# Michaelszeng/GCS-ADMM

Measured on NVIDIA B200. Metric: admm_iterations_per_second, higher is better.
Workload: dtype f64

## Files before the change

gcs-admm_b200/build.py:

```python
from __future__ import annotations

import os
import shutil
import subprocess
import sys

HERE = os.path.dirname(os.path.abspath(__file__))
SRC = os.path.join(HERE, "csrc", "gcsadmm.cu")


def deps():
    import glob
    return sorted(glob.glob(os.path.join(HERE, "csrc", "*.cu")) + glob.glob(os.path.join(HERE, "csrc", "*.cuh"))
                  + glob.glob(os.path.join(os.path.dirname(HERE), "include", "*.h")))


OUT = os.path.join(HERE, "libgcsadmm.so")


def nvcc_path():
    for cand in (shutil.which("nvcc"), "/usr/local/cuda/bin/nvcc"):
        if cand and os.path.exists(cand):
            return cand
    raise RuntimeError("nvcc not found: libgcsadmm.so cannot be built")


def build(force=False, verbose=False):
    if not force and os.path.exists(OUT) and all(os.path.getmtime(OUT) >= os.path.getmtime(d) for d in deps()):
        return OUT
    cmd = [nvcc_path(), "-gencode", "arch=compute_100a,code=sm_100a", "-lineinfo", "-O3", "-std=c++17",
           "-Xptxas", "-v", "-shared", "-Xcompiler", "-fPIC", "-ccbin", "/usr/bin/g++", "-o", OUT, SRC]
    r = subprocess.run(cmd, capture_output=True, text=True)
    if verbose or r.returncode != 0:
        sys.stderr.write(r.stdout + r.stderr)
    if r.returncode != 0:
        raise RuntimeError("nvcc failed building libgcsadmm.so")
    with open(os.path.join(HERE, "csrc", "ptxas_info.txt"), "w") as fh:
        fh.write(r.stderr)
    return OUT


if __name__ == "__main__":
    print(build(force=True, verbose=True))
```

gcs-admm_b200/csrc/gcsadmm.cu:

```cuda
#include <cuda_runtime.h>
#include <math.h>
#include <stdio.h>
#include <stdlib.h>
#include <string.h>
#include <new>
#include <nvtx3/nvToolsExt.h>

struct NvtxRange {
    explicit NvtxRange(const char *name) { nvtxRangePushA(name); }
    ~NvtxRange() { nvtxRangePop(); }
};

#include "../../include/gcsadmm.h"
#include "gcs_ctrl.h"
#include "vertex_update.cuh"
#include "vertex_perf.cuh"

#define GCS_VERSION "gcsadmm 0.1.0 (sm_100a)"
#define K1_MAX_WARPS 12
#define EDGE_THREADS 256

static thread_local char g_err[512] = "";
static int set_err(int code, const char *fmt, const char *a = "", const char *b = "") {
    snprintf(g_err, sizeof g_err, fmt, a, b);
// ... 68 lines not shown
vertex_kernel(GcsGraphView G, GcsStateView St, Ctrl *ctrl_all, const int *__restrict__ vprob, GcsScratchLayout L, double tol, int max_iter) {
    extern __shared__ double smem[];
    const int lane = threadIdx.x & 31, warp = threadIdx.x >> 5;
    const int v = blockIdx.x * (blockDim.x >> 5) + warp;
    if (v >= G.nV) return;
    Ctrl *ctrl = ctrl_all + (vprob ? vprob[v] : 0);
    if (ctrl->stop && !ctrl->ignore_stop) return;
    double *S = smem + (size_t)warp * L.total;
    int status = 0;
    const int iters = gcs_vertex_update(G, St, v, ctrl->rho, ctrl->mu_scale, tol, max_iter, L, S, lane, &status);
    if (lane == 0) {
        if (iters) atomicAdd(&ctrl->inner_iters, (unsigned long long)iters);
        if (status > 0 && status != 5) atomicAdd(&ctrl->inner_fail, 1);
        if (status < 0) atomicAdd(&ctrl->skipped, 1ull);
    }
}

__device__ __forceinline__ unsigned long long gcs_globaltimer() { unsigned long long t; asm volatile("mov.u64 %0, %globaltimer;" : "=l"(t)); return t; }

__device__ __forceinline__ void peer_push(const double *xc, const int *__restrict__ send_he, const int *__restrict__ send_rank,
                                          const int *__restrict__ send_slot, int nsend, const PeerView &PV) {
    const int k = PV.comm[PV.rank]->k + 1, par = k & 1;
    for (int i = threadIdx.x; i < 5 * nsend; i += blockDim.x) {
        const int j = i / 5, c = i - 5 * j, q = send_rank[j];
        PV.xc[q][5 * ((size_t)PV.nHown[q] + (size_t)par * PV.nHghost[q] + send_slot[j]) + c] = __ldcg(xc + 5 * (size_t)send_he[j] + c);
    }
    __threadfence_system();
    __syncthreads();
    if (threadIdx.x < PV.world && ((PV.neighbours >> threadIdx.x) & 1u)) *(volatile int *)&PV.comm[threadIdx.x]->halo_flag[PV.rank] = k;
}
__device__ __forceinline__ void peer_wait_halo(const PeerView &PV) {
    PeerComm *me = PV.comm[PV.rank];
    const int k = me->k + 1, p = threadIdx.x;
    if (p < PV.world && ((PV.neighbours >> p) & 1u)) {
        const unsigned long long t0 = gcs_globaltimer();
        while (*(volatile int *)&me->halo_flag[p] < k)
            if (gcs_globaltimer() - t0 > GCS_PEER_TIMEOUT_NS) { me->error = 1; break; }
        __threadfence_system();
    }
    __syncthreads();
}

template <bool INNER, bool BATCH>
__global__ void __launch_bounds__(GCS_PERF_THREADS, 4)
vertex_perf_kernel(GcsGraphView G, GcsStateView St, GcsPerfTables T, Ctrl *ctrl_all, GcsPerfLayout L, PeerPush P) {
    extern __shared__ __align__(16) double smem[];
    __shared__ __align__(8) unsigned long long bar[2];
    if (!BATCH) {
        if (ctrl_all->stop && !ctrl_all->ignore_stop) return;
        if (blockIdx.x == 0 && threadIdx.x == 0) atomicAdd(&ctrl_all->inner_iters, (unsigned long long)T.inner_iters * (unsigned long long)G.nV);
    }
    int tile = blockIdx.x;
    if (tile >= T.ntiles) return;
    double *const stage0 = smem + L.work;
#define STAGE(b) (stage0 + (b) * L.stage)
    if (threadIdx.x == 0) {
        gcs_mbar_init(&bar[0], 1);
        gcs_mbar_init(&bar[1], 1);
        gcs_perf_stage(T, L, STAGE(0), tile, &bar[0]);
    }
    __syncthreads();
    double rin = 0.0;
    for (unsigned n = 0; tile < T.ntiles; tile += gridDim.x, ++n) {
        const int buf = n & 1;
        gcs_mbar_wait(&bar[buf], (n >> 1) & 1u);
        gcs_perf_tile<INNER, BATCH>(G, St, T, L, smem, STAGE(buf), tile, ctrl_all, rin, STAGE(buf ^ 1), tile + gridDim.x, &bar[buf ^ 1]);
    }
    if (threadIdx.x == GCS_COPY_THREAD) gcs_bulk_wait_read();
#undef STAGE
    if (INNER) {
#pragma unroll
        for (int o = 16; o; o >>= 1) rin += __shfl_xor_sync(0xffffffffu, rin, o);
        __syncthreads();
        if ((threadIdx.x & 31) == 0) smem[L.rin + (threadIdx.x >> 5)] = rin;
        __syncthreads();
        if (threadIdx.x == 0) {
            double s = 0.0;
            for (int w2 = 0; w2 < (int)(blockDim.x >> 5); ++w2) s += smem[L.rin + w2];
            T.tile_res[blockIdx.x] = s;
        }
    }
    if (P.PV) {
        __shared__ int is_last;
        __threadfence();
        __syncthreads();
        if (threadIdx.x == 0) is_last = (atomicAdd(P.ticket, 1u) == gridDim.x - 1);
        __syncthreads();
        if (is_last) {
            __threadfence();
            peer_push(St.xc, P.send_he, P.send_rank, P.send_slot, P.nsend, *P.PV);
            if (threadIdx.x == 0) *P.ticket = 0u;
        }
    }
}
__global__ void perf_init_dead_kernel(GcsGraphView G, GcsStateView St) {
    const int v = blockIdx.x * blockDim.x + threadIdx.x;
    if (v >= G.nV || G.vtype[v] != GCS_VT_DEAD) return;
    for (int k = 0; k < 4; ++k) { St.z_v[4 * (size_t)v + k] = 0.0; St.x_v[4 * (size_t)v + k] = G.cent[2 * (size_t)v + (k & 1)]; }
    St.y_v[v] = 0.0;
}

__device__ void control_apply(Ctrl *ctrl, const GcsParams &p, long long n_x, long long n_mu, double *hist, int hist_cap) {
    const int it = ctrl->it + 1;
    const double *s = ctrl->sums;
    const double rho = ctrl->rho;
    const double pri = sqrt(s[0]);
    const double dual = rho * sqrt(2.0 * s[1]);
    double rho_new = rho, scale = 1.0;
    const bool may = it < p.frac * p.max_it && (p.adapt_every <= 1 || it % p.adapt_every == 0);
    if (pri >= p.nu * dual && may) { rho_new = rho * p.tau_incr; scale = 1.0 / p.tau_incr; }
    else if (dual >= p.nu * pri && may) { rho_new = rho * (1.0 / p.tau_decr); scale = p.tau_incr; }
    const double nAx = sqrt(s[2]), nBz = sqrt(2.0 * s[3]), nmu = scale * sqrt(s[4]);
    const double eps_pri = sqrt((double)n_x) * p.eps_abs + p.eps_rel * fmax(nAx, nBz);
    const double eps_dual = sqrt((double)n_mu) * p.eps_abs + p.eps_rel * nmu;
    const double inner = s[6] < 0.0 ? -1.0 : sqrt(s[6]);
    const double pri_g = s[7] < 0.0 ? -1.0 : sqrt(s[7]), dual_g = s[8] < 0.0 ? -1.0 : rho * sqrt(2.0 * s[8]);
    ctrl->pri_g = pri_g; ctrl->dual_g = dual_g;
    ctrl->it = it; ctrl->pri = pri; ctrl->dual = dual; ctrl->eps_pri = eps_pri; ctrl->eps_dual = eps_dual; ctrl->inner = inner;
    ctrl->rho = rho_new; ctrl->mu_scale = scale;
    if (it < hist_cap) { hist[it] = rho_new; hist[hist_cap + it] = pri; hist[2 * hist_cap + it] = dual; }
// ... 994 lines not shown
                        if (gb < g || (gb == 2) != (bb == c->blk_off[v + 1] - 1)) rc = set_err(GCS_E_INVALID, "perf-mode blocks of a vertex are not in-, out-, z-block order%s", "");
                        g = gb; nin += gb == 0;
                    }
                    int *w = vrec + GCS_VI_N * (size_t)v;
                    w[GCS_VI_CONE] = c->cone_off[v] - c->cone_off[a]; w[GCS_VI_NV] = c->cone_off[v + 1] - c->cone_off[v];
                    w[GCS_VI_CLS] = c->vclass[v]; w[GCS_VI_TERM] = (vtype[v] != GCS_VT_GENERIC) | (nin << 1);
                    w[GCS_VI_BLK] = c->blk_off[v] - c->blk_off[a]; w[GCS_VI_NB] = c->blk_off[v + 1] - c->blk_off[v];
                    w[GCS_VI_ACTIVE] = vprob[v]; w[GCS_VI_HE] = he_off[v] - he_off[a];
                }
            }
            if (!rc) rc = upload(&h->p_blk_rec, brec, 4 * nB);
            if (!rc) rc = upload(&h->p_vrec, vrec, GCS_VI_N * nVt);
            if (!rc) rc = upload(&h->p_tile_rec, trec, 8 * nT);
        }
        free(brec); free(vrec); free(trec); free(he_edge); free(he_off); free(vtype); free(he_flags); free(vprob);
    }
    if (!rc) rc = upload(&h->p_tstate, (const double *)nullptr, 12 * (size_t)c->n_blocks);
    if (!rc) rc = upload(&h->p_tn, (const double *)nullptr, 2 * (size_t)h->nV);
    if (!rc) rc = upload(&h->p_tile_res, (const double *)nullptr, (size_t)c->n_tiles);
    if (!rc && c->edge_delta) rc = upload(&h->p_edge_delta, c->edge_delta, 2 * (size_t)h->nE);
    if (!rc && c->edge_delta && c->edge_cent) rc = upload(&h->p_edge_cent, c->edge_cent, 2 * (size_t)h->nE);
    if (rc) { free_perf(h); return rc; }
    h->perf_nblocks = c->n_blocks;
    h->PL = gcs_perf_layout(c->cap_blocks, c->cap_verts, c->cap_cone);
    h->PT.vclass = h->p_vclass; h->PT.cls_tab = h->p_cls_tab; h->PT.cone_off = h->p_cone_off; h->PT.cone = h->p_cone;
    h->PT.blk_off = h->p_blk_off; h->PT.blk_rec = h->p_blk_rec; h->PT.vrec = h->p_vrec; h->PT.tile_rec = h->p_tile_rec;
    h->PT.ntiles = c->n_tiles; h->PT.tstate = h->p_tstate; h->PT.tn = h->p_tn; h->PT.inner_iters = c->inner_iters;
    h->PT.alpha = c->alpha; h->PT.kappa = c->kappa; h->PT.theta = c->theta > 0.0 ? c->theta : 1.0; h->PT.edge_delta = h->p_edge_delta; h->PT.tile_res = h->p_tile_res;
    cudaDeviceProp prop;
    CK(cudaGetDeviceProperties(&prop, h->device));
    const size_t bytes = (size_t)(h->PL.work + 2 * h->PL.stage) * sizeof(double);
    if (bytes > prop.sharedMemPerBlockOptin) { free_perf(h); return set_err(GCS_E_INVALID, "perf-mode tile too large for shared memory (a vertex of very high degree)%s", ""); }
    h->perf_smem = (int)bytes;
    h->perf_threads = c->threads >= 32 && c->threads <= GCS_PERF_THREADS ? (c->threads / 32) * 32 : GCS_PERF_THREADS;
    {
        const char *bps = getenv("GCS_PERF_BLOCKS_PER_SM");
        int per_sm = bps && atoi(bps) > 0 ? atoi(bps) : 4;
        const int by_smem = (int)(prop.sharedMemPerMultiprocessor / (bytes + 1024));
        if (per_sm > by_smem) per_sm = by_smem > 0 ? by_smem : 1;
        const long long cap = (long long)prop.multiProcessorCount * per_sm;
        h->perf_grid = (int)(c->n_tiles < cap ? c->n_tiles : cap);
    }
    for (auto *k : {vertex_perf_kernel<false, false>, vertex_perf_kernel<true, false>, vertex_perf_kernel<false, true>, vertex_perf_kernel<true, true>}) {
        CK(cudaFuncSetAttribute(k, cudaFuncAttributeMaxDynamicSharedMemorySize, h->perf_smem));
        CK(cudaFuncSetAttribute(k, cudaFuncAttributePreferredSharedMemoryCarveout, 100));
    }
    perf_init_dead_kernel<<<(h->nV + 255) / 256, 256, 0, h->stream>>>(graph_view(h), state_view(h));
    CK(cudaGetLastError());
    CK(cudaStreamSynchronize(h->stream));
    h->perf_on = 1;
    return 0;
}

extern "C" int gcsadmm_get_perf_state(GcsHandle *h, double *tstate, double *tn) {
    if (!h || !h->perf_on) return set_err(GCS_E_INVALID, "perf mode is not enabled%s", "");
    CK(cudaSetDevice(h->device));
    CK(cudaStreamSynchronize(h->stream));
    if (tstate && h->perf_nblocks) CK(cudaMemcpy(tstate, h->p_tstate, sizeof(double) * 12 * (size_t)h->perf_nblocks, cudaMemcpyDeviceToHost));
    if (tn) CK(cudaMemcpy(tn, h->p_tn, sizeof(double) * 2 * (size_t)h->nV, cudaMemcpyDeviceToHost));
    return 0;
}
extern "C" int gcsadmm_set_perf_state(GcsHandle *h, const double *tstate, const double *tn) {
    if (!h || !h->perf_on) return set_err(GCS_E_INVALID, "perf mode is not enabled%s", "");
    CK(cudaSetDevice(h->device));
    CK(cudaStreamSynchronize(h->stream));
    if (tstate && h->perf_nblocks) CK(cudaMemcpy(h->p_tstate, tstate, sizeof(double) * 12 * (size_t)h->perf_nblocks, cudaMemcpyHostToDevice));
    if (tn) CK(cudaMemcpy(h->p_tn, tn, sizeof(double) * 2 * (size_t)h->nV, cudaMemcpyHostToDevice));
    return 0;
}
```

gcs-admm_b200/csrc/vertex_perf.cuh:

```cuda
#pragma once
#include <string.h>
#include "gcs_ctrl.h"
#include "vertex_update.cuh"

#define GCS_CONE_REC 12
#define GCS_NCX 19
#define GCS_CLS_G0 361
#define GCS_CLS_DINV 380
#define GCS_CLS_STRIDE 392
#define GCS_PERF_THREADS 256

#ifdef GCS_EMULATE
#define GCS_CTA_LOOP(i, n) for (int i = 0; i < (n); ++i)
#define GCS_CTA_SYNC() ((void)0)
#else
#define GCS_CTA_LOOP(i, n) for (int i = threadIdx.x; i < (n); i += blockDim.x)
#define GCS_CTA_SYNC() __syncthreads()
#endif

struct GcsPerfTables {
    const int *vclass;
    const double *cls_tab;
    const int *cone_off;
    const double *cone;
// ... 102 lines not shown
        if (dist > 0.0) gcs_cone_take_face(gcs_cone_sector_dot(cone, k, 0, c0, c1, c2) >= 0.0 && gcs_cone_sector_dot(cone, k, 1, c0, c1, c2) >= 0.0, k, best, code, inside);
    }
    gcs_cone_pick(cone, code, inside, c0, c1, c2, q0, q1, q2);
}
GCS_DEV void gcs_cone_project2(const double *cone, int nv, double c0, double c1, double c2, double d0, double d1, double d2,
                               double &q0, double &q1, double &q2, double &s0, double &s1, double &s2) {
    double best_c = 0.0, best_d = 0.0;
    int code_c = -1, code_d = -1;
    bool inside_c = true, inside_d = true;
#pragma unroll 1
    for (int k = 0; k < nv; ++k) {
        const GcsConeRay R = gcs_cone_ray(cone, k);
        const double dist_c = gcs_cone_test_ray(R, k, c0, c1, c2, best_c, code_c);
        const double dist_d = gcs_cone_test_ray(R, k, d0, d1, d2, best_d, code_d);
        if (dist_c > 0.0 || dist_d > 0.0) {
            const bool ma_c = gcs_cone_sector_dot(cone, k, 0, c0, c1, c2) >= 0.0, ma_d = gcs_cone_sector_dot(cone, k, 0, d0, d1, d2) >= 0.0;
            const bool mb_c = gcs_cone_sector_dot(cone, k, 1, c0, c1, c2) >= 0.0, mb_d = gcs_cone_sector_dot(cone, k, 1, d0, d1, d2) >= 0.0;
            if (dist_c > 0.0) gcs_cone_take_face(ma_c && mb_c, k, best_c, code_c, inside_c);
            if (dist_d > 0.0) gcs_cone_take_face(ma_d && mb_d, k, best_d, code_d, inside_d);
        }
    }
    gcs_cone_pick(cone, code_c, inside_c, c0, c1, c2, q0, q1, q2);
    gcs_cone_pick(cone, code_d, inside_d, d0, d1, d2, s0, s1, s2);
}

#if !defined(GCS_EMULATE) && defined(__CUDACC__)
__device__ __forceinline__ unsigned gcs_smem_u32(const void *p) { return (unsigned)__cvta_generic_to_shared(p); }
__device__ __forceinline__ void gcs_mbar_init(unsigned long long *bar, unsigned count) {
    asm volatile("mbarrier.init.shared::cta.b64 [%0], %1;" ::"r"(gcs_smem_u32(bar)), "r"(count) : "memory");
    asm volatile("fence.mbarrier_init.release.cluster;" ::: "memory");
}
__device__ __forceinline__ void gcs_mbar_expect_tx(unsigned long long *bar, unsigned bytes) {
    asm volatile("mbarrier.arrive.expect_tx.shared::cta.b64 _, [%0], %1;" ::"r"(gcs_smem_u32(bar)), "r"(bytes) : "memory");
}
__device__ __forceinline__ void gcs_bulk_g2s(void *dst, const void *src, unsigned bytes, unsigned long long *bar) {
    asm volatile("cp.async.bulk.shared::cluster.global.mbarrier::complete_tx::bytes [%0], [%1], %2, [%3];"
                 ::"r"(gcs_smem_u32(dst)), "l"(src), "r"(bytes), "r"(gcs_smem_u32(bar)) : "memory");
}
__device__ __forceinline__ void gcs_mbar_wait(unsigned long long *bar, unsigned parity) {
    unsigned done = 0;
    while (!done) {
        asm volatile("{\n .reg .pred p;\n mbarrier.try_wait.parity.shared::cta.b64 p, [%1], %2;\n selp.u32 %0, 1, 0, p;\n}"
                     : "=r"(done) : "r"(gcs_smem_u32(bar)), "r"(parity) : "memory");
    }
}
__device__ __forceinline__ void gcs_bulk_s2g(void *dst, const void *src, unsigned bytes) {
    asm volatile("cp.async.bulk.global.shared::cta.bulk_group [%0], [%1], %2;" ::"l"(dst), "r"(gcs_smem_u32(src)), "r"(bytes) : "memory");
}
__device__ __forceinline__ void gcs_bulk_commit() { asm volatile("cp.async.bulk.commit_group;" ::: "memory"); }
__device__ __forceinline__ void gcs_bulk_wait_read() { asm volatile("cp.async.bulk.wait_group.read 0;" ::: "memory"); }
__device__ __forceinline__ void gcs_fence_async_smem() { asm volatile("fence.proxy.async.shared::cta;" ::: "memory"); }
#endif

#define GCS_PF 3

GCS_DEV double gcs_core_input(const double *tS, const double *rS, const int *w, int k, double kappa) {
    const int bl = w[GCS_VI_BLK], zb = bl + w[GCS_VI_NB] - 1;
    double s = 0.0;
    if (k < 4) {
        if (!(w[GCS_VI_TERM] & 1)) { for (int b = bl; b <= zb; ++b) s += tS[12 * b + 6 * (k >> 1) + 3 + (k & 1)]; s *= kappa; }
    } else if (k < 9) s = rS[5 * zb + k - 4];
    else {
        const int g = k >= 14, tau = k - 9 - 5 * g, bin = bl + (w[GCS_VI_TERM] >> 1);
        for (int b = g ? bin : bl; b < (g ? zb : bin); ++b) s += rS[5 * b + tau];
    }
    return s;
}
GCS_DEV double gcs_core_output(const double *tab, const double *in, int k) {
    const double *gk = tab + k;
    double s0 = tab[GCS_CLS_G0 + k], s1 = 0.0;
#pragma unroll
    for (int j = 0; j + 1 < GCS_NCX; j += 2) { s0 += gk[GCS_NCX * j] * in[j]; s1 += gk[GCS_NCX * (j + 1)] * in[j + 1]; }
    return s0 + s1 + gk[GCS_NCX * (GCS_NCX - 1)] * in[GCS_NCX - 1];
}

GCS_DEV double gcs_rhs(const GcsPerfTables &T, const double *tS, const double *TS, const double *tnS, const int *brec, int q, int vl, double rho, double kappa) {
    const int b = q / 5, tau = q - 5 * b, info = brec[4 * b + 1], grp = (info >> 8) & 3;
    const bool term = (info >> 10) & 1;
    const double *d = tS + 12 * b;
    double val;
    if (tau < 4) {
        const int i = tau >> 1, c = tau & 1;
        val = d[6 * i + c];
        if (!term) val -= d[6 * i + 3 + c];
        val *= kappa;
        if (grp == 1) val += TS[q];
        else if (grp == 0) { if (tau < 2) val += TS[q + 2]; }
        else val += (i ? -kappa : kappa) * tnS[2 * vl + c];
    } else {
        val = d[2] + d[8];
        if (!term) val += (1.0 - d[5]) + (1.0 - d[11]);
        val *= kappa;
        if (grp < 2) val += T.theta * TS[q] - GCS_EDGE_PENALTY / rho;
    }
    return val;
}
GCS_DEV double gcs_block_u(const double *rS, const double *co, const double *tab, int info, int b, int tau) {
    const int grp = (info >> 8) & 3;
    return grp == 2 ? co[4 + tau] : tab[GCS_CLS_DINV + 5 * grp + tau] * rS[5 * b + tau] + co[9 + 5 * grp + tau];
}

GCS_DEV double gcs_target_z(const GcsStateView &St, const GcsPerfTables &T, int e, int c, int info) {
    double zc = St.z[5 * (size_t)e + c];
    if (T.edge_delta && ((info >> 8) & 3) == 1 && (c == 2 || c == 3))
        zc -= T.edge_delta[2 * (size_t)e + c - 2] * St.z[5 * (size_t)e + 4];
    return zc;
}


#if !defined(GCS_EMULATE) && defined(__CUDACC__)
#define GCS_COPY_THREAD (blockDim.x - 32)
__device__ __forceinline__ void gcs_perf_stage(const GcsPerfTables &T, const GcsPerfLayout &L, double *B, int tile, unsigned long long *bar) {
    const int *tr = T.tile_rec + 8 * (size_t)tile;
    const int v0 = tr[0], nvt = tr[1], b0 = tr[2], nb = tr[3], c0 = tr[4], ncone = tr[5];
    gcs_mbar_expect_tx(bar, (unsigned)(sizeof(double) * (12 * nb + 2 * nvt + GCS_CONE_REC * ncone) + sizeof(int) * (GCS_VI_N * nvt + 4 * nb + 8)));
    gcs_bulk_g2s(B + L.tr, tr, (unsigned)(sizeof(int) * 8), bar);
    gcs_bulk_g2s(B + L.vi, T.vrec + GCS_VI_N * (size_t)v0, (unsigned)(sizeof(int) * GCS_VI_N * nvt), bar);
    if (nb) gcs_bulk_g2s(B + L.bi, T.blk_rec + 4 * (size_t)b0, (unsigned)(sizeof(int) * 4 * nb), bar);
    if (nb) gcs_bulk_g2s(B + L.tS, T.tstate + 12 * (size_t)b0, (unsigned)(sizeof(double) * 12 * nb), bar);
    gcs_bulk_g2s(B + L.tnS, T.tn + 2 * (size_t)v0, (unsigned)(sizeof(double) * 2 * nvt), bar);
    if (ncone) gcs_bulk_g2s(B + L.cone, T.cone + GCS_CONE_REC * (size_t)c0, (unsigned)(sizeof(double) * GCS_CONE_REC * ncone), bar);
}
#endif

GCS_DEV void gcs_cstep_store(double *t, double *e, double t0, double t1, double t2, double q0, double q1, double q2, double ms, double alpha) {
    const double l0 = ms * (t0 - q0), l1 = ms * (t1 - q1), l2 = ms * (t2 - q2);
    t[0] = q0 - l0; t[1] = q1 - l1; t[2] = q2 - l2;
    e[0] = (1.0 - alpha) * q0 + l0; e[1] = (1.0 - alpha) * q1 + l1; e[2] = (1.0 - alpha) * q2 + l2;
}

template <bool INNER, bool BATCH>
GCS_DEV void gcs_perf_tile(const GcsGraphView &G, const GcsStateView &St, const GcsPerfTables &T, const GcsPerfLayout &L,
                           double *S, double *B, int tile, Ctrl *ctrl_all, double &rin,
                           double *Bn, int next, unsigned long long *bar_next) {
    const double rho_u = ctrl_all->rho, ms_u = ctrl_all->mu_scale;
#define RHO(vl) (BATCH ? vd[2 * (vl)] : rho_u)
#define MSC(vl) (BATCH ? vd[2 * (vl) + 1] : ms_u)
#define ACT(vl) (!BATCH || vi[GCS_VI_N * (vl) + GCS_VI_ACTIVE])
#define ACT_W (!BATCH || w[GCS_VI_ACTIVE])
#if defined(GCS_EMULATE)
    const int *tr = T.tile_rec + 8 * (size_t)tile;
#else
    const int *tr = (const int *)(B + L.tr);
#endif
    const int v0 = tr[0], nvt = tr[1], b0 = tr[2], nb = tr[3], h0 = tr[6], nhe = tr[7] & 0x3fffffff;
    const bool has_zero = (tr[7] >> 30) & 1;
    double *tS = B + L.tS, *eS = S + L.eS, *coneS = B + L.cone, *tnS = B + L.tnS, *enS = S + L.enS, *TS = S + L.T, *rS = S + L.r;
    double *cin = S + L.cin, *cout = S + L.cout, *vd = S + L.vd;
    int *vi = (int *)(B + L.vi), *brec = (int *)(B + L.bi);
#define bhe(b) brec[4 * (b)]
#define binfo(b) brec[4 * (b) + 1]
#define bedge(b) brec[4 * (b) + 2]
#if defined(GCS_EMULATE)
    {
        const int c0 = tr[4], ncone = tr[5];
        memcpy(tS, T.tstate + 12 * (size_t)b0, sizeof(double) * 12 * nb);
        memcpy(tnS, T.tn + 2 * (size_t)v0, sizeof(double) * 2 * nvt);
        memcpy(coneS, T.cone + GCS_CONE_REC * (size_t)c0, sizeof(double) * GCS_CONE_REC * ncone);
        memcpy(vi, T.vrec + GCS_VI_N * (size_t)v0, sizeof(int) * GCS_VI_N * nvt);
        memcpy(brec, T.blk_rec + 4 * (size_t)b0, sizeof(int) * 4 * nb);
    }
#endif
#if defined(GCS_EMULATE)
    const bool cgrp = true, ggrp = true;
    const int cid = 0, cn = 1, gid0 = 0, gn = 1;
#else
    const int nw = blockDim.x >> 5, cn = 32 * ((nw + 1) >> 1);
    const bool cgrp = (int)threadIdx.x < cn, ggrp = !cgrp || nw == 1;
    const int cid = threadIdx.x, gid0 = nw == 1 ? (int)threadIdx.x : (int)threadIdx.x - cn, gn = nw == 1 ? cn : (int)blockDim.x - cn;
#endif
    if (BATCH) {
        GCS_CTA_LOOP(i, nvt) {
            int *w = vi + GCS_VI_N * i;
            Ctrl *c = ctrl_all + w[GCS_VI_ACTIVE];
            w[GCS_VI_ACTIVE] = !(c->stop && !c->ignore_stop);
            vd[2 * i] = c->rho; vd[2 * i + 1] = c->mu_scale;
            if (w[GCS_VI_ACTIVE] && w[GCS_VI_NB]) {
#if defined(GCS_EMULATE)
                c->inner_iters += (unsigned long long)T.inner_iters;
#else
                atomicAdd(&c->inner_iters, (unsigned long long)T.inner_iters);
#endif
            }
        }
        GCS_CTA_SYNC();
    }
    const double alpha = T.alpha, kappa = T.kappa;
    for (int it = 0; it < T.inner_iters; ++it) {
        const bool last = it + 1 == T.inner_iters;
        if (ggrp) {
#if defined(GCS_EMULATE)
            const int gid = gid0;
#else
            int gid = gid0;
            asm volatile("" : "+r"(gid));
#endif
            if (it == 0 && has_zero) for (int q = gid; q < 5 * nhe; q += gn) {
                const int hl = q / 5, c = q - 5 * hl, h = h0 + hl, f = G.he_flags[h];
                if (!(f & GCS_HE_ZERO)) continue;
                int vl = 0;
                while (vl + 1 < nvt && vi[GCS_VI_N * (vl + 1) + GCS_VI_HE] <= hl) ++vl;
                if (!ACT(vl)) continue;
                double x = 0.0;
                if (c < 2 && !(f & GCS_HE_OUT)) x = St.z[5 * (size_t)G.he_edge[h] + c] + MSC(vl) * St.mu[5 * (size_t)h + c];
                St.xc[5 * (size_t)h + c] = x;
            }
            for (int i = gid; i < nvt; i += gn) {
                const int *w = vi + GCS_VI_N * i;
                if (!ACT_W || !w[GCS_VI_NB]) continue;
                const double ms = it ? 1.0 : MSC(i);
                const double sigma = kappa * RHO(i) * ms;
                const double a0 = tnS[2 * i], a1 = tnS[2 * i + 1], nrm = hypot(a0, a1);
                const double sc = nrm > 0.0 ? fmax(0.0, 1.0 - 1.0 / (sigma * nrm)) : 0.0;
                const double q0 = sc * a0, q1 = sc * a1, l0 = ms * (a0 - q0), l1 = ms * (a1 - q1);
                tnS[2 * i] = q0 - l0; tnS[2 * i + 1] = q1 - l1;
                enS[2 * i] = (1.0 - alpha) * q0 + l0; enS[2 * i + 1] = (1.0 - alpha) * q1 + l1;
            }
#if !defined(GCS_EMULATE)
            double pz[GCS_PF], pm[GCS_PF];
            if (it == 0) {
#pragma unroll
                for (int j = 0; j < GCS_PF; ++j) {
                    const int q = gid + j * gn;
                    pz[j] = 0.0; pm[j] = 0.0;
                    if (q < 5 * nb) {
                        const int b = q / 5, c = q - 5 * b, h = bhe(b);
                        if (h >= 0) { pz[j] = gcs_target_z(St, T, bedge(b), c, binfo(b)); pm[j] = St.mu[5 * (size_t)h + c]; }
                    }
                }
            }
#endif
            if (it == 0) {
#if !defined(GCS_EMULATE)
#pragma unroll
                for (int j = 0; j < GCS_PF; ++j) {
                    const int q = gid + j * gn;
                    if (q < 5 * nb) TS[q] = pz[j] + MSC(binfo(q / 5) & 255) * pm[j];
                }
                for (int q = gid + GCS_PF * gn; q < 5 * nb; q += gn) {
#else
                for (int q = 0; q < 5 * nb; ++q) {
#endif
                    const int b = q / 5, c = q - 5 * b, h = bhe(b), vl = binfo(b) & 255;
                    if (h < 0 || !ACT(vl)) continue;
                    TS[q] = gcs_target_z(St, T, bedge(b), c, binfo(b)) + MSC(vl) * St.mu[5 * (size_t)h + c];
                }
            }
        }
        if (cgrp) for (int j = cid; j < 2 * nb; j += cn) {
            const int b = j >> 1, info = binfo(b), vl = info & 255;
            const int *w = vi + GCS_VI_N * vl;
            if (!ACT_W) continue;
            const double ms = it ? 1.0 : MSC(vl);
            const double *cone = coneS + GCS_CONE_REC * w[GCS_VI_CONE];
            double *t = tS + 6 * j, *e = eS + 6 * j;
            const double t0 = t[0], t1 = t[1], t2 = t[2];
            double q0, q1, q2;
            if ((info >> 10) & 1) gcs_cone_project(cone, w[GCS_VI_NV], t0, t1, t2, q0, q1, q2);
            else {
                const double t3 = t[3], t4 = t[4], t5 = t[5];
                double q3, q4, q5;
                gcs_cone_project2(cone, w[GCS_VI_NV], t0, t1, t2, t3, t4, t5, q0, q1, q2, q3, q4, q5);
                gcs_cstep_store(t + 3, e + 3, t3, t4, t5, q3, q4, q5, ms, alpha);
            }
            gcs_cstep_store(t, e, t0, t1, t2, q0, q1, q2, ms, alpha);
        }
        GCS_CTA_SYNC();
#if !defined(GCS_EMULATE)
        if (it == 0 && threadIdx.x == GCS_COPY_THREAD && next < T.ntiles) {
            gcs_bulk_wait_read();
            gcs_perf_stage(T, L, Bn, next, bar_next);
        }
#endif
#if defined(GCS_EMULATE)
        for (int vl = 0; vl < nvt; ++vl) {
            const int *w = vi + GCS_VI_N * vl;
            if (!ACT_W || !w[GCS_VI_NB]) continue;
            for (int q = 5 * w[GCS_VI_BLK]; q < 5 * (w[GCS_VI_BLK] + w[GCS_VI_NB]); ++q) rS[q] = gcs_rhs(T, tS, TS, tnS, brec, q, vl, RHO(vl), kappa);
            for (int k = 0; k < GCS_NCX; ++k) cin[GCS_NCX * vl + k] = gcs_core_input(tS, rS, w, k, kappa);
            for (int k = 0; k < GCS_NCX; ++k) cout[GCS_NCX * vl + k] = gcs_core_output(T.cls_tab + (size_t)GCS_CLS_STRIDE * w[GCS_VI_CLS], cin + GCS_NCX * vl, k);
        }
#else
        for (int vl = threadIdx.x >> 5; vl < nvt; vl += blockDim.x >> 5) {
            const int *w = vi + GCS_VI_N * vl;
            const int k = threadIdx.x & 31;
            if (!ACT_W || !w[GCS_VI_NB]) continue;
            for (int q = 5 * w[GCS_VI_BLK] + k; q < 5 * (w[GCS_VI_BLK] + w[GCS_VI_NB]); q += 32) rS[q] = gcs_rhs(T, tS, TS, tnS, brec, q, vl, RHO(vl), kappa);
            __syncwarp();
            if (k < GCS_NCX) cin[GCS_NCX * vl + k] = gcs_core_input(tS, rS, w, k, kappa);
            __syncwarp();
            if (k < GCS_NCX) cout[GCS_NCX * vl + k] = gcs_core_output(T.cls_tab + (size_t)GCS_CLS_STRIDE * w[GCS_VI_CLS], cin + GCS_NCX * vl, k);
        }
#endif
        GCS_CTA_SYNC();
        GCS_CTA_LOOP(p, 4 * nb) {
            const int b = p >> 2, i = (p >> 1) & 1, fam = p & 1, info = binfo(b), vl = info & 255;
            const int *w = vi + GCS_VI_N * vl;
            if (!ACT_W || ((info >> 10) & fam)) continue;
            const double *co = cout + GCS_NCX * vl, *tab = T.cls_tab + (size_t)GCS_CLS_STRIDE * w[GCS_VI_CLS], *e = eS + 3 * p;
            double p0 = gcs_block_u(rS, co, tab, info, b, 2 * i), p1 = gcs_block_u(rS, co, tab, info, b, 2 * i + 1), p2 = gcs_block_u(rS, co, tab, info, b, 4);
            if (fam) { p0 = co[2 * i] - p0; p1 = co[2 * i + 1] - p1; p2 = 1.0 - p2; }
            double *t = tS + 3 * p;
            if (INNER && last) {
                const double ic = 1.0 / (2.0 - alpha), r0 = p0 - ic * (t[0] + e[0]), r1 = p1 - ic * (t[1] + e[1]), r2_ = p2 - ic * (t[2] + e[2]);
                rin += r0 * r0 + r1 * r1 + r2_ * r2_;
            }
            t[0] = alpha * p0 + e[0]; t[1] = alpha * p1 + e[1]; t[2] = alpha * p2 + e[2];
        }
        GCS_CTA_LOOP(i, nvt) {
            const int *w = vi + GCS_VI_N * i;
            if (!ACT_W || !w[GCS_VI_NB]) continue;
            const double *zz = cout + GCS_NCX * i + 4;
            if (INNER && last) {
                const double ic = 1.0 / (2.0 - alpha), r0 = (zz[0] - zz[2]) - ic * (tnS[2 * i] + enS[2 * i]), r1 = (zz[1] - zz[3]) - ic * (tnS[2 * i + 1] + enS[2 * i + 1]);
                rin += r0 * r0 + r1 * r1;
            }
            tnS[2 * i] = alpha * (zz[0] - zz[2]) + enS[2 * i]; tnS[2 * i + 1] = alpha * (zz[1] - zz[3]) + enS[2 * i + 1];
        }
        if (last) {
            GCS_CTA_LOOP(q, 9 * nvt) {
                const int vl = q / 9, k = q - 9 * vl;
                const int *w = vi + GCS_VI_N * vl;
                if (!ACT_W || !w[GCS_VI_NB]) continue;
                double val = cout[GCS_NCX * vl + k];
                const size_t v = (size_t)(v0 + vl);
                if (T.edge_delta && k < 8)
                    val += (k < 4 ? 1.0 : cout[GCS_NCX * vl + 8]) * G.cent[2 * v + (k & 1)];
                if (k < 4) St.x_v[4 * v + k] = val; else if (k < 8) St.z_v[4 * v + k - 4] = val; else St.y_v[v] = val;
            }
            GCS_CTA_LOOP(q, 5 * nb) {
                const int b = q / 5, c = q - 5 * b, h = bhe(b), info = binfo(b), vl = info & 255;
                const int *w = vi + GCS_VI_N * vl;
                if (h < 0 || !ACT_W) continue;
                const double *co = cout + GCS_NCX * vl, *tab = T.cls_tab + (size_t)GCS_CLS_STRIDE * w[GCS_VI_CLS];
                double x;
                if ((info >> 8) & 1) x = gcs_block_u(rS, co, tab, info, b, c);
                else x = c < 2 ? TS[q] : gcs_block_u(rS, co, tab, info, b, c < 4 ? c - 2 : 4);
                St.xc[5 * (size_t)h + c] = x;
            }
        }
        if (!last) GCS_CTA_SYNC();
    }
#if defined(GCS_EMULATE)
    memcpy(T.tstate + 12 * (size_t)b0, tS, sizeof(double) * 12 * nb);
    memcpy(T.tn + 2 * (size_t)v0, tnS, sizeof(double) * 2 * nvt);
#else
    gcs_fence_async_smem();
    GCS_CTA_SYNC();
    if (threadIdx.x == GCS_COPY_THREAD) {
        if (nb) gcs_bulk_s2g(T.tstate + 12 * (size_t)b0, tS, (unsigned)(sizeof(double) * 12 * nb));
        gcs_bulk_s2g(T.tn + 2 * (size_t)v0, tnS, (unsigned)(sizeof(double) * 2 * nvt));
        gcs_bulk_commit();
    }
#endif
#undef bhe
#undef binfo
#undef bedge
#undef RHO
#undef MSC
#undef ACT
#undef ACT_W
}
```

gcs-admm_b200/lib.py:

```python
from __future__ import annotations

import ctypes as C
import os

import numpy as np

from . import build as _build

_dp = np.ctypeslib.ndpointer(dtype=np.float64, flags="C_CONTIGUOUS")

EXPORTS = [
    "gcsadmm_version", "gcsadmm_last_error", "gcsadmm_device_count", "gcsadmm_default_params",
    "gcsadmm_create", "gcsadmm_destroy", "gcsadmm_set_stream", "gcsadmm_run", "gcsadmm_step",
    "gcsadmm_get_status", "gcsadmm_vertex_update", "gcsadmm_edge_update", "gcsadmm_control",
    "gcsadmm_sums_device_ptr", "gcsadmm_xc_device_ptr", "gcsadmm_get_history", "gcsadmm_get_solution",
    "gcsadmm_get_state", "gcsadmm_set_state", "gcsadmm_time_steps", "gcsadmm_time_window", "gcsadmm_solve_host",
    "gcsadmm_scratch_bytes", "gcsadmm_flush_l2", "gcsadmm_get_problem_status", "gcsadmm_get_problem_history", "gcsadmm_enable_perf",
    "gcsadmm_get_perf_state", "gcsadmm_set_perf_state", "gcsadmm_peer_export", "gcsadmm_peer_connect", "gcsadmm_peer_error",
]


class GcsGraph(C.Structure):
    _fields_ = [("nV", C.c_int32), ("nE", C.c_int32), ("n", C.c_int32), ("nH_own", C.c_int32), ("nH_ghost", C.c_int32),
                ("poly_off", C.c_void_p), ("polyA", C.c_void_p), ("polyb", C.c_void_p),
                ("he_off", C.c_void_p), ("he_edge", C.c_void_p), ("he_flags", C.c_void_p),
                ("edge_he_tail", C.c_void_p), ("edge_he_head", C.c_void_p), ("edge_counted", C.c_void_p),
                ("vtype", C.c_void_p), ("cent", C.c_void_p),
                ("n_x_global", C.c_int64), ("n_mu_global", C.c_int64),
                ("nP", C.c_int32), ("prob_voff", C.c_void_p), ("prob_eoff", C.c_void_p)]


class GcsParams(C.Structure):
    _fields_ = [("rho0", C.c_double), ("tau_incr", C.c_double), ("tau_decr", C.c_double), ("nu", C.c_double),
                ("frac", C.c_double), ("eps_abs", C.c_double), ("eps_rel", C.c_double), ("max_it", C.c_int32),
                ("inner_tol", C.c_double), ("inner_max_iter", C.c_int32), ("check_every", C.c_int32),
                ("abs_stop", C.c_int32), ("abs_tol", C.c_double), ("warm_theta", C.c_double), ("zero_tol", C.c_double),
                ("outer_alpha", C.c_double), ("use_graph", C.c_int32), ("adapt_every", C.c_int32), ("stop_ref", C.c_int32)]


class GcsPerfConfig(C.Structure):
    _fields_ = [("inner_iters", C.c_int32), ("alpha", C.c_double), ("kappa", C.c_double), ("n_classes", C.c_int32),
                ("vclass", C.c_void_p), ("cls_tab", C.c_void_p), ("cone_off", C.c_void_p), ("cone", C.c_void_p),
                ("n_blocks", C.c_int32), ("blk_off", C.c_void_p), ("blk_he", C.c_void_p), ("blk_info", C.c_void_p),
                ("n_tiles", C.c_int32), ("tile_voff", C.c_void_p),
                ("cap_blocks", C.c_int32), ("cap_verts", C.c_int32), ("cap_cone", C.c_int32), ("threads", C.c_int32),
                ("theta", C.c_double), ("edge_delta", C.c_void_p), ("edge_cent", C.c_void_p)]


class GcsStatus(C.Structure):
    _fields_ = [("iterations", C.c_int32), ("converged", C.c_int32), ("diverged", C.c_int32),
                ("inner_fail", C.c_int32), ("inner_iters", C.c_int64), ("skipped", C.c_int64), ("rho", C.c_double), ("pri_res", C.c_double),
                ("dual_res", C.c_double), ("eps_pri", C.c_double), ("eps_dual", C.c_double), ("inner_res", C.c_double),
                ("pri_res_ref", C.c_double), ("dual_res_ref", C.c_double)]

    def as_dict(self):
        return {k: getattr(self, k) for k, _ in self._fields_}


_LIB = None


def library_path():
    return os.path.join(os.path.dirname(os.path.abspath(__file__)), "libgcsadmm.so")


def load():
    global _LIB
    if _LIB is not None:
        return _LIB
    path = _build.build()
    L = C.CDLL(path)
    L.gcsadmm_version.restype = C.c_char_p
    L.gcsadmm_last_error.restype = C.c_char_p
    L.gcsadmm_default_params.argtypes = [C.POINTER(GcsParams)]
    L.gcsadmm_default_params.restype = None
    L.gcsadmm_create.argtypes = [C.POINTER(GcsGraph), C.POINTER(GcsParams), C.c_int, C.POINTER(C.c_void_p)]
    L.gcsadmm_destroy.argtypes = [C.c_void_p]
    L.gcsadmm_set_stream.argtypes = [C.c_void_p, C.c_void_p, C.c_int]
    L.gcsadmm_run.argtypes = [C.c_void_p, C.c_int, C.POINTER(GcsStatus)]
    L.gcsadmm_step.argtypes = [C.c_void_p, C.c_int]
    L.gcsadmm_get_status.argtypes = [C.c_void_p, C.POINTER(GcsStatus)]
    L.gcsadmm_get_problem_status.argtypes = [C.c_void_p, C.c_int, C.POINTER(GcsStatus)]
    L.gcsadmm_get_problem_history.argtypes = [C.c_void_p, C.c_int, C.c_void_p, C.c_void_p, C.c_void_p, C.c_int]
    for f in ("gcsadmm_vertex_update", "gcsadmm_edge_update", "gcsadmm_control"):
        getattr(L, f).argtypes = [C.c_void_p]
    L.gcsadmm_sums_device_ptr.argtypes = [C.c_void_p, C.POINTER(C.c_void_p)]
    L.gcsadmm_xc_device_ptr.argtypes = [C.c_void_p, C.POINTER(C.c_void_p)]
    L.gcsadmm_get_history.argtypes = [C.c_void_p, C.c_void_p, C.c_void_p, C.c_void_p, C.c_int]
    L.gcsadmm_get_solution.argtypes = [C.c_void_p, C.c_void_p, C.c_void_p, C.c_void_p, C.c_void_p]
    L.gcsadmm_get_state.argtypes = [C.c_void_p, C.c_void_p, C.c_void_p, C.c_void_p, C.POINTER(C.c_double), C.POINTER(C.c_int)]
    L.gcsadmm_set_state.argtypes = [C.c_void_p, C.c_void_p, C.c_void_p, C.c_void_p, C.c_double, C.c_int]
    L.gcsadmm_time_steps.argtypes = [C.c_void_p, C.c_int, C.POINTER(C.c_float), C.POINTER(C.c_float), C.POINTER(C.c_float)]
    L.gcsadmm_time_window.argtypes = [C.c_void_p, C.c_int, C.c_longlong, C.c_void_p, C.c_void_p]
    L.gcsadmm_solve_host.argtypes = [C.POINTER(GcsGraph), C.POINTER(GcsParams), C.c_int, C.c_int, C.POINTER(GcsStatus),
                                     C.c_void_p, C.c_void_p, C.c_void_p, C.c_void_p, C.c_void_p, C.c_void_p, C.c_void_p, C.c_int]
    L.gcsadmm_enable_perf.argtypes = [C.c_void_p, C.POINTER(GcsPerfConfig)]
    L.gcsadmm_get_perf_state.argtypes = [C.c_void_p, C.c_void_p, C.c_void_p]
    L.gcsadmm_set_perf_state.argtypes = [C.c_void_p, C.c_void_p, C.c_void_p]
    L.gcsadmm_peer_export.argtypes = [C.c_void_p, C.c_void_p]
    L.gcsadmm_peer_connect.argtypes = [C.c_void_p, C.c_int, C.c_int, C.c_void_p, C.c_void_p, C.c_void_p, C.c_int, C.c_void_p, C.c_void_p, C.c_void_p]
    L.gcsadmm_peer_error.argtypes = [C.c_void_p]
    L.gcsadmm_scratch_bytes.argtypes = [C.c_int, C.c_int]
    L.gcsadmm_flush_l2.argtypes = [C.c_void_p, C.c_longlong]
    _LIB = L
    return L


class GcsError(RuntimeError):
    def __init__(self, code, msg):
        super().__init__(f"libgcsadmm error {code}: {msg}")
        self.code = code


GCS_E_DIVERGED = -4


def _check(rc, allow_diverged=False):
    if rc < 0 and not (allow_diverged and rc == GCS_E_DIVERGED):
        raise GcsError(rc, load().gcsadmm_last_error().decode())
    return rc


def default_params(**overrides):
# ... 229 lines not shown
```

Before: 4040.

## Fuse block-u and output writes into per-vertex warp loop; add phase clock probes

Restructures the per-vertex warp loop so that each lane computes all five rhs entries for a block at once, loading the 12-value tstate record as double2 vectors. The same lane then computes the block solution u in place in rS, and on the last iteration writes xc and the vertex outputs directly. The later phase reads the precomputed u instead of recomputing gcs_block_u, and the separate final-iteration output loops are removed. Optional clock64 phase instrumentation is added behind a compile define, along with build and load hooks for alternate builds. Parallelism per vertex moves from per-rhs-entry to per-block, which may lower lane utilisation for vertices with few blocks.

Result: faster. 4183, median of 6 (+3.5%).

```diff
diff --git a/gcs-admm_b200/build.py b/gcs-admm_b200/build.py
--- a/gcs-admm_b200/build.py
+++ b/gcs-admm_b200/build.py
@@ -25,19 +25,20 @@
     raise RuntimeError("nvcc not found: libgcsadmm.so cannot be built")
 
 
-def build(force=False, verbose=False):
-    if not force and os.path.exists(OUT) and all(os.path.getmtime(OUT) >= os.path.getmtime(d) for d in deps()):
-        return OUT
+def build(force=False, verbose=False, out=OUT, defines=()):
+    if not force and os.path.exists(out) and all(os.path.getmtime(out) >= os.path.getmtime(d) for d in deps()):
+        return out
     cmd = [nvcc_path(), "-gencode", "arch=compute_100a,code=sm_100a", "-lineinfo", "-O3", "-std=c++17",
-           "-Xptxas", "-v", "-shared", "-Xcompiler", "-fPIC", "-ccbin", "/usr/bin/g++", "-o", OUT, SRC]
+           "-Xptxas", "-v", "-shared", "-Xcompiler", "-fPIC", "-ccbin", "/usr/bin/g++", *[f"-D{d}" for d in defines], "-o", out, SRC]
     r = subprocess.run(cmd, capture_output=True, text=True)
     if verbose or r.returncode != 0:
         sys.stderr.write(r.stdout + r.stderr)
     if r.returncode != 0:
-        raise RuntimeError("nvcc failed building libgcsadmm.so")
-    with open(os.path.join(HERE, "csrc", "ptxas_info.txt"), "w") as fh:
-        fh.write(r.stderr)
-    return OUT
+        raise RuntimeError(f"nvcc failed building {os.path.basename(out)}")
+    if out == OUT:
+        with open(os.path.join(HERE, "csrc", "ptxas_info.txt"), "w") as fh:
+            fh.write(r.stderr)
+    return out
 
 
 if __name__ == "__main__":
diff --git a/gcs-admm_b200/csrc/gcsadmm.cu b/gcs-admm_b200/csrc/gcsadmm.cu
--- a/gcs-admm_b200/csrc/gcsadmm.cu
+++ b/gcs-admm_b200/csrc/gcsadmm.cu
@@ -144,6 +144,7 @@
     }
     int tile = blockIdx.x;
     if (tile >= T.ntiles) return;
+    GCS_PHASE(if (long long *ph = gcs_phase_row()) ph[GCS_PH_MARK] = 0;)
     double *const stage0 = smem + L.work;
 #define STAGE(b) (stage0 + (b) * L.stage)
     if (threadIdx.x == 0) {
@@ -158,6 +159,7 @@
         gcs_mbar_wait(&bar[buf], (n >> 1) & 1u);
         gcs_perf_tile<INNER, BATCH>(G, St, T, L, smem, STAGE(buf), tile, ctrl_all, rin, STAGE(buf ^ 1), tile + gridDim.x, &bar[buf ^ 1]);
     }
+    GCS_PHASE(if (long long *ph = gcs_phase_row()) { ph[GCS_PH_P8] += clock64() - ph[GCS_PH_MARK]; ph[GCS_PH_MARK] = 0; })
     if (threadIdx.x == GCS_COPY_THREAD) gcs_bulk_wait_read();
 #undef STAGE
     if (INNER) {
@@ -1258,6 +1260,18 @@
     return 0;
 }
 
+#if defined(GCS_PHASE_CLOCKS)
+extern "C" int gcsadmm_phase_clocks(GcsHandle *h, long long *out, int cap) {
+    if (!h || !h->perf_on) return set_err(GCS_E_INVALID, "perf mode is not enabled%s", "");
+    CK(cudaSetDevice(h->device));
+    CK(cudaStreamSynchronize(h->stream));
+    const int n = h->perf_grid < cap ? h->perf_grid : cap, rows = n < GCS_PH_GRID ? n : GCS_PH_GRID;
+    CK(cudaMemcpyFromSymbol(out, gcs_phase_clk, sizeof(long long) * GCS_PH_N * rows));
+    static const long long zero[GCS_PH_GRID][GCS_PH_N] = {};
+    CK(cudaMemcpyToSymbol(gcs_phase_clk, zero, sizeof(zero)));
+    return h->perf_grid;
+}
+#endif
 extern "C" int gcsadmm_get_perf_state(GcsHandle *h, double *tstate, double *tn) {
     if (!h || !h->perf_on) return set_err(GCS_E_INVALID, "perf mode is not enabled%s", "");
     CK(cudaSetDevice(h->device));
diff --git a/gcs-admm_b200/csrc/vertex_perf.cuh b/gcs-admm_b200/csrc/vertex_perf.cuh
--- a/gcs-admm_b200/csrc/vertex_perf.cuh
+++ b/gcs-admm_b200/csrc/vertex_perf.cuh
@@ -178,6 +178,21 @@
 __device__ __forceinline__ void gcs_fence_async_smem() { asm volatile("fence.proxy.async.shared::cta;" ::: "memory"); }
 #endif
 
+#if defined(GCS_PHASE_CLOCKS) && !defined(GCS_EMULATE)
+enum { GCS_PH_CSTEP, GCS_PH_GATHER, GCS_PH_P12, GCS_PH_P36, GCS_PH_P7, GCS_PH_P8, GCS_PH_TILES, GCS_PH_MARK, GCS_PH_N };
+#define GCS_PH_GRID 4096
+__device__ long long gcs_phase_clk[GCS_PH_GRID][GCS_PH_N];
+__device__ __forceinline__ long long *gcs_phase_row() { return threadIdx.x == 0 && blockIdx.x < GCS_PH_GRID ? gcs_phase_clk[blockIdx.x] : nullptr; }
+__device__ __forceinline__ long long gcs_phase_add(long long *ph, int k, long long since) {
+    const long long now = clock64();
+    if (ph) ph[k] += now - since;
+    return now;
+}
+#define GCS_PHASE(...) __VA_ARGS__
+#else
+#define GCS_PHASE(...)
+#endif
+
 #define GCS_PF 3
 
 GCS_DEV double gcs_core_input(const double *tS, const double *rS, const int *w, int k, double kappa) {
@@ -200,30 +215,60 @@
     return s0 + s1 + gk[GCS_NCX * (GCS_NCX - 1)] * in[GCS_NCX - 1];
 }
 
-GCS_DEV double gcs_rhs(const GcsPerfTables &T, const double *tS, const double *TS, const double *tnS, const int *brec, int q, int vl, double rho, double kappa) {
-    const int b = q / 5, tau = q - 5 * b, info = brec[4 * b + 1], grp = (info >> 8) & 3;
+#if defined(GCS_EMULATE)
+GCS_DEV double gcs_mul_rn(double a, double b) { return a * b; }
+GCS_DEV double gcs_fma_rn(double a, double b, double c) { return a * b + c; }
+#else
+GCS_DEV double gcs_mul_rn(double a, double b) { return __dmul_rn(a, b); }
+GCS_DEV double gcs_fma_rn(double a, double b, double c) { return __fma_rn(a, b, c); }
+#endif
+GCS_DEV void gcs_rhs(const GcsPerfTables &T, const double *tS, const double *TS, const double *tnS, int b, int info, int vl, double rho, double kappa, double *r) {
+    const int grp = (info >> 8) & 3;
     const bool term = (info >> 10) & 1;
-    const double *d = tS + 12 * b;
-    double val;
-    if (tau < 4) {
+    double d[12];
+#if defined(GCS_EMULATE)
+    memcpy(d, tS + 12 * b, sizeof d);
+#else
+    const double2 *d2 = reinterpret_cast<const double2 *>(tS + 12 * b);
+#pragma unroll
+    for (int j = 0; j < 6; ++j) { const double2 v = d2[j]; d[2 * j] = v.x; d[2 * j + 1] = v.y; }
+#endif
+    const double *Tb = TS + 5 * b;
+#pragma unroll
+    for (int tau = 0; tau < 4; ++tau) {
         const int i = tau >> 1, c = tau & 1;
-        val = d[6 * i + c];
+        double val = d[6 * i + c];
         if (!term) val -= d[6 * i + 3 + c];
-        val *= kappa;
-        if (grp == 1) val += TS[q];
-        else if (grp == 0) { if (tau < 2) val += TS[q + 2]; }
-        else val += (i ? -kappa : kappa) * tnS[2 * vl + c];
-    } else {
-        val = d[2] + d[8];
-        if (!term) val += (1.0 - d[5]) + (1.0 - d[11]);
-        val *= kappa;
-        if (grp < 2) val += T.theta * TS[q] - GCS_EDGE_PENALTY / rho;
-    }
-    return val;
-}
-GCS_DEV double gcs_block_u(const double *rS, const double *co, const double *tab, int info, int b, int tau) {
+        val = gcs_mul_rn(val, kappa);
+        if (grp == 1) val += Tb[tau];
+        else if (grp == 0) { if (tau < 2) val += Tb[tau + 2]; }
+        else val = gcs_fma_rn(i ? -kappa : kappa, tnS[2 * vl + c], val);
+        r[tau] = val;
+    }
+    double val = d[2] + d[8];
+    if (!term) val += (1.0 - d[5]) + (1.0 - d[11]);
+    val = gcs_mul_rn(val, kappa);
+    if (grp < 2) val += T.theta * Tb[4] - GCS_EDGE_PENALTY / rho;
+    r[4] = val;
+}
+GCS_DEV void gcs_block_u(double *r, const double *co, const double *tab, int info, double *u) {
     const int grp = (info >> 8) & 3;
-    return grp == 2 ? co[4 + tau] : tab[GCS_CLS_DINV + 5 * grp + tau] * rS[5 * b + tau] + co[9 + 5 * grp + tau];
+#pragma unroll
+    for (int tau = 0; tau < 5; ++tau) {
+        u[tau] = grp == 2 ? co[4 + tau] : tab[GCS_CLS_DINV + 5 * grp + tau] * r[tau] + co[9 + 5 * grp + tau];
+        r[tau] = u[tau];
+    }
+}
+GCS_DEV void gcs_block_xc(const GcsStateView &St, int h, int info, const double *u, const double *Tb) {
+    double *x = St.xc + 5 * (size_t)h;
+    if ((info >> 8) & 1) { x[0] = u[0]; x[1] = u[1]; x[2] = u[2]; x[3] = u[3]; x[4] = u[4]; }
+    else { x[0] = Tb[0]; x[1] = Tb[1]; x[2] = u[0]; x[3] = u[1]; x[4] = u[4]; }
+}
+GCS_DEV void gcs_vertex_out(const GcsGraphView &G, const GcsStateView &St, const GcsPerfTables &T, const double *co, size_t v, int k) {
+    double val = co[k];
+    if (T.edge_delta && k < 8)
+        val += (k < 4 ? 1.0 : co[8]) * G.cent[2 * v + (k & 1)];
+    if (k < 4) St.x_v[4 * v + k] = val; else if (k < 8) St.z_v[4 * v + k - 4] = val; else St.y_v[v] = val;
 }
 
 GCS_DEV double gcs_target_z(const GcsStateView &St, const GcsPerfTables &T, int e, int c, int info) {
@@ -287,6 +332,8 @@
         memcpy(brec, T.blk_rec + 4 * (size_t)b0, sizeof(int) * 4 * nb);
     }
 #endif
+    GCS_PHASE(long long *const ph = gcs_phase_row(); long long mk = clock64();
+              if (ph) { if (ph[GCS_PH_MARK]) ph[GCS_PH_P8] += mk - ph[GCS_PH_MARK]; ++ph[GCS_PH_TILES]; })
 #if defined(GCS_EMULATE)
     const bool cgrp = true, ggrp = true;
     const int cid = 0, cn = 1, gid0 = 0, gn = 1;
@@ -314,6 +361,7 @@
     const double alpha = T.alpha, kappa = T.kappa;
     for (int it = 0; it < T.inner_iters; ++it) {
         const bool last = it + 1 == T.inner_iters;
+        GCS_PHASE(const long long p0 = clock64();)
         if (ggrp) {
 #if defined(GCS_EMULATE)
             const int gid = gid0;
@@ -373,6 +421,7 @@
                 }
             }
         }
+        GCS_PHASE(if (!cgrp && gid0 == 0 && blockIdx.x < GCS_PH_GRID) gcs_phase_clk[blockIdx.x][GCS_PH_GATHER] += clock64() - p0;)
         if (cgrp) for (int j = cid; j < 2 * nb; j += cn) {
             const int b = j >> 1, info = binfo(b), vl = info & 255;
             const int *w = vi + GCS_VI_N * vl;
@@ -391,7 +440,9 @@
             }
             gcs_cstep_store(t, e, t0, t1, t2, q0, q1, q2, ms, alpha);
         }
+        GCS_PHASE(gcs_phase_add(ph, GCS_PH_CSTEP, p0);)
         GCS_CTA_SYNC();
+        GCS_PHASE(mk = gcs_phase_add(ph, GCS_PH_P12, mk);)
 #if !defined(GCS_EMULATE)
         if (it == 0 && threadIdx.x == GCS_COPY_THREAD && next < T.ntiles) {
             gcs_bulk_wait_read();
@@ -402,30 +453,46 @@
         for (int vl = 0; vl < nvt; ++vl) {
             const int *w = vi + GCS_VI_N * vl;
             if (!ACT_W || !w[GCS_VI_NB]) continue;
-            for (int q = 5 * w[GCS_VI_BLK]; q < 5 * (w[GCS_VI_BLK] + w[GCS_VI_NB]); ++q) rS[q] = gcs_rhs(T, tS, TS, tnS, brec, q, vl, RHO(vl), kappa);
+            const double *tab = T.cls_tab + (size_t)GCS_CLS_STRIDE * w[GCS_VI_CLS];
+            for (int b = w[GCS_VI_BLK]; b < w[GCS_VI_BLK] + w[GCS_VI_NB]; ++b) gcs_rhs(T, tS, TS, tnS, b, binfo(b), vl, RHO(vl), kappa, rS + 5 * b);
             for (int k = 0; k < GCS_NCX; ++k) cin[GCS_NCX * vl + k] = gcs_core_input(tS, rS, w, k, kappa);
-            for (int k = 0; k < GCS_NCX; ++k) cout[GCS_NCX * vl + k] = gcs_core_output(T.cls_tab + (size_t)GCS_CLS_STRIDE * w[GCS_VI_CLS], cin + GCS_NCX * vl, k);
+            for (int k = 0; k < GCS_NCX; ++k) cout[GCS_NCX * vl + k] = gcs_core_output(tab, cin + GCS_NCX * vl, k);
+            for (int b = w[GCS_VI_BLK]; b < w[GCS_VI_BLK] + w[GCS_VI_NB]; ++b) {
+                double u[5];
+                gcs_block_u(rS + 5 * b, cout + GCS_NCX * vl, tab, binfo(b), u);
+                if (last && bhe(b) >= 0) gcs_block_xc(St, bhe(b), binfo(b), u, TS + 5 * b);
+            }
+            if (last) for (int k = 0; k < 9; ++k) gcs_vertex_out(G, St, T, cout + GCS_NCX * vl, (size_t)(v0 + vl), k);
         }
 #else
         for (int vl = threadIdx.x >> 5; vl < nvt; vl += blockDim.x >> 5) {
             const int *w = vi + GCS_VI_N * vl;
-            const int k = threadIdx.x & 31;
-            if (!ACT_W || !w[GCS_VI_NB]) continue;
-            for (int q = 5 * w[GCS_VI_BLK] + k; q < 5 * (w[GCS_VI_BLK] + w[GCS_VI_NB]); q += 32) rS[q] = gcs_rhs(T, tS, TS, tnS, brec, q, vl, RHO(vl), kappa);
+            const int k = threadIdx.x & 31, bl = w[GCS_VI_BLK], be = bl + w[GCS_VI_NB];
+            if (!ACT_W || bl == be) continue;
+            const double *tab = T.cls_tab + (size_t)GCS_CLS_STRIDE * w[GCS_VI_CLS];
+            for (int b = bl + k; b < be; b += 32) gcs_rhs(T, tS, TS, tnS, b, binfo(b), vl, RHO(vl), kappa, rS + 5 * b);
             __syncwarp();
             if (k < GCS_NCX) cin[GCS_NCX * vl + k] = gcs_core_input(tS, rS, w, k, kappa);
             __syncwarp();
-            if (k < GCS_NCX) cout[GCS_NCX * vl + k] = gcs_core_output(T.cls_tab + (size_t)GCS_CLS_STRIDE * w[GCS_VI_CLS], cin + GCS_NCX * vl, k);
+            if (k < GCS_NCX) cout[GCS_NCX * vl + k] = gcs_core_output(tab, cin + GCS_NCX * vl, k);
+            __syncwarp();
+            for (int b = bl + k; b < be; b += 32) {
+                double u[5];
+                gcs_block_u(rS + 5 * b, cout + GCS_NCX * vl, tab, binfo(b), u);
+                if (last && bhe(b) >= 0) gcs_block_xc(St, bhe(b), binfo(b), u, TS + 5 * b);
+            }
+            if (last && k < 9) gcs_vertex_out(G, St, T, cout + GCS_NCX * vl, (size_t)(v0 + vl), k);
         }
 #endif
         GCS_CTA_SYNC();
+        GCS_PHASE(mk = gcs_phase_add(ph, GCS_PH_P36, mk);)
         GCS_CTA_LOOP(p, 4 * nb) {
             const int b = p >> 2, i = (p >> 1) & 1, fam = p & 1, info = binfo(b), vl = info & 255;
             const int *w = vi + GCS_VI_N * vl;
             if (!ACT_W || ((info >> 10) & fam)) continue;
-            const double *co = cout + GCS_NCX * vl, *tab = T.cls_tab + (size_t)GCS_CLS_STRIDE * w[GCS_VI_CLS], *e = eS + 3 * p;
-            double p0 = gcs_block_u(rS, co, tab, info, b, 2 * i), p1 = gcs_block_u(rS, co, tab, info, b, 2 * i + 1), p2 = gcs_block_u(rS, co, tab, info, b, 4);
-            if (fam) { p0 = co[2 * i] - p0; p1 = co[2 * i + 1] - p1; p2 = 1.0 - p2; }
+            const double *u = rS + 5 * b, *e = eS + 3 * p;
+            double p0 = u[2 * i], p1 = u[2 * i + 1], p2 = u[4];
+            if (fam) { const double *co = cout + GCS_NCX * vl; p0 = co[2 * i] - p0; p1 = co[2 * i + 1] - p1; p2 = 1.0 - p2; }
             double *t = tS + 3 * p;
             if (INNER && last) {
                 const double ic = 1.0 / (2.0 - alpha), r0 = p0 - ic * (t[0] + e[0]), r1 = p1 - ic * (t[1] + e[1]), r2_ = p2 - ic * (t[2] + e[2]);
@@ -443,30 +510,10 @@
             }
             tnS[2 * i] = alpha * (zz[0] - zz[2]) + enS[2 * i]; tnS[2 * i + 1] = alpha * (zz[1] - zz[3]) + enS[2 * i + 1];
         }
-        if (last) {
-            GCS_CTA_LOOP(q, 9 * nvt) {
-                const int vl = q / 9, k = q - 9 * vl;
-                const int *w = vi + GCS_VI_N * vl;
-                if (!ACT_W || !w[GCS_VI_NB]) continue;
-                double val = cout[GCS_NCX * vl + k];
-                const size_t v = (size_t)(v0 + vl);
-                if (T.edge_delta && k < 8)
-                    val += (k < 4 ? 1.0 : cout[GCS_NCX * vl + 8]) * G.cent[2 * v + (k & 1)];
-                if (k < 4) St.x_v[4 * v + k] = val; else if (k < 8) St.z_v[4 * v + k - 4] = val; else St.y_v[v] = val;
-            }
-            GCS_CTA_LOOP(q, 5 * nb) {
-                const int b = q / 5, c = q - 5 * b, h = bhe(b), info = binfo(b), vl = info & 255;
-                const int *w = vi + GCS_VI_N * vl;
-                if (h < 0 || !ACT_W) continue;
-                const double *co = cout + GCS_NCX * vl, *tab = T.cls_tab + (size_t)GCS_CLS_STRIDE * w[GCS_VI_CLS];
-                double x;
-                if ((info >> 8) & 1) x = gcs_block_u(rS, co, tab, info, b, c);
-                else x = c < 2 ? TS[q] : gcs_block_u(rS, co, tab, info, b, c < 4 ? c - 2 : 4);
-                St.xc[5 * (size_t)h + c] = x;
-            }
-        }
+        GCS_PHASE(mk = gcs_phase_add(ph, GCS_PH_P7, mk);)
         if (!last) GCS_CTA_SYNC();
     }
+    GCS_PHASE(if (ph) ph[GCS_PH_MARK] = mk;)
 #if defined(GCS_EMULATE)
     memcpy(T.tstate + 12 * (size_t)b0, tS, sizeof(double) * 12 * nb);
     memcpy(T.tn + 2 * (size_t)v0, tnS, sizeof(double) * 2 * nvt);
diff --git a/gcs-admm_b200/lib.py b/gcs-admm_b200/lib.py
--- a/gcs-admm_b200/lib.py
+++ b/gcs-admm_b200/lib.py
@@ -64,11 +64,11 @@
     return os.path.join(os.path.dirname(os.path.abspath(__file__)), "libgcsadmm.so")
 
 
-def load():
+def load(path=None):
     global _LIB
     if _LIB is not None:
         return _LIB
-    path = _build.build()
+    path = path or _build.build()
     L = C.CDLL(path)
     L.gcsadmm_version.restype = C.c_char_p
     L.gcsadmm_last_error.restype = C.c_char_p
```
